# inhavl-shlee/AFI-GAN

Measured on AMD Instinct MI355X. Metric: stage1_G+D_step_images_per_s, higher is better.
Workload: dtype f32 via f16x3: two scaled fp16 pieces per operand, three f16 MFMAs per product, fp32 accumulate (tensors fp32)

## Files before the change

afigan_amd/_lib.py:

```python
import ctypes as C
import os
import re

import torch

_HERE = os.path.dirname(os.path.abspath(__file__))
LIB_PATH = os.environ.get("AFI_LIB_PATH") or os.path.join(_HERE, "csrc", "libafigan_hip.so")

HEADER_PATH = os.path.join(os.path.dirname(_HERE), "include", "afigan_hip.h")
ABI_VERSION = 9


class AfiError(RuntimeError):
    pass


def _strip_comments(text):
    return re.sub(r"/\*.*?\*/|//[^\n]*", " ", text, flags=re.S)


def parse_defines(text):
    raw = dict(re.findall(r"^[ \t]*#[ \t]*define[ \t]+(AFI_\w+)[ \t]+(\w+)[ \t]*$", _strip_comments(text), flags=re.M))
    try:
        return {k: int(raw.get(v, v), 0) for k, v in raw.items()}
# ... 17 lines not shown
    _fields_ = [("p", C.c_void_p), ("sN", C.c_longlong), ("sH", C.c_longlong), ("sW", C.c_longlong)]


class GenParams(C.Structure):
    _fields_ = [("C", C.c_int), ("G", C.c_int), ("n_rdb", C.c_int), ("residual_scale", C.c_float),
                ("w0", C.c_void_p), ("b0", C.c_void_p),
                ("rdb_w", (C.c_void_p * 5) * AFI_MAX_RDB),
                ("w7", C.c_void_p), ("b7", C.c_void_p),
                ("wT", C.c_void_p), ("bT", C.c_void_p),
                ("w9", C.c_void_p), ("b9", C.c_void_p)]


class DiscParams(C.Structure):
    _fields_ = [("F", C.c_int * 4),
                ("w", C.c_void_p * 3), ("b", C.c_void_p * 3),
                ("gamma", C.c_void_p * 3), ("beta", C.c_void_p * 3),
                ("running_mean", C.c_void_p * 3), ("running_var", C.c_void_p * 3),
                ("num_batches_tracked", C.c_void_p * 3),
                ("w3", C.c_void_p), ("b3", C.c_void_p)]


class SgdDesc(C.Structure):
    _fields_ = [("p", C.c_void_p), ("g", C.c_void_p), ("m", C.c_void_p), ("n", C.c_longlong),
                ("wd", C.c_float), ("pad_", C.c_float)]


class UnfoldDesc(C.Structure):
    _fields_ = [("dw", C.c_void_p), ("grad", C.c_void_p), ("s", C.c_void_p), ("O", C.c_int), ("I", C.c_int), ("k", C.c_int), ("pad_", C.c_int)]


class DetSgdDesc(C.Structure):
    _fields_ = [("p", C.c_void_p), ("g", C.c_void_p), ("m", C.c_void_p), ("n", C.c_longlong), ("lr", C.c_float), ("wd", C.c_float),
                ("fold_out", C.c_void_p), ("s64", C.c_void_p), ("O", C.c_int), ("I", C.c_int), ("k", C.c_int), ("pad_", C.c_int)]


_CTYPES = {"int": C.c_int, "long long": C.c_longlong, "float": C.c_float, "double": C.c_double, "afi_view_t": View,
           "const afi_gen_params_t*": C.POINTER(GenParams), "const afi_disc_params_t*": C.POINTER(DiscParams), "const char*": C.c_char_p}


def _ctype(decl, where):
    t = " ".join(decl.replace("*", " * ").split()).replace(" *", "*")
    if t in _CTYPES:
        return _CTYPES[t]
    if t.endswith("*"):
        return C.c_void_p
    raise AfiError(f"{HEADER_PATH}: {where}: no ctypes type for {t!r} (the binding knows {sorted(_CTYPES)} and pointers)")


def parse_prototypes(text):
    text = re.sub(r"^[ \t]*#.*$", " ", _strip_comments(text), flags=re.M)
    text = re.sub(r"typedef\s+struct\s+\w*\s*\{[^}]*\}\s*\w+\s*;|typedef[^;{]*;|extern\s+\"C\"\s*\{", " ", text)
    sigs = {}
    for ret, name, args in re.findall(r"([\w\s\*]+?)\b(afi_\w+)\s*\(([^()]*)\)\s*;", text):
        args = [a.strip() for a in args.split(",")] if args.strip() not in ("", "void") else []
        sigs[name] = (_ctype(ret, name), [C.c_void_p if "[" in a else _ctype(re.sub(r"\w+$", "", a), f"{name}({a})") for a in args])
    return sigs


SIGNATURES = parse_prototypes(_HEADER)

_lib = None


def load():
    global _lib
    if _lib is not None:
# ... 177 lines not shown
```

afigan_amd/csrc/nets.hip:

```cpp
#include <string.h>
#include <stdlib.h>

#include "../../include/afigan_hip.h"
#include "afi_common.h"
#include "afi_launch.h"
#include <initializer_list>
#include <new>


#include <vector>
namespace {
struct SideStream {
    hipStream_t side = nullptr;
    std::vector<hipEvent_t> ring;
    size_t next = 0;
    bool init() {
        if (side) return true;
        if (hipStreamCreateWithFlags(&side, hipStreamNonBlocking) != hipSuccess) { side = nullptr; return false; }
        ring.resize(128);
        for (auto& e : ring)
            if (hipEventCreateWithFlags(&e, hipEventDisableTiming) != hipSuccess) return false;
        return true;
    }
    void destroy() {
// ... 277 lines not shown
    if (P > kWk6MaxPixels || !wk6_shapes_ok(C, G, R)) return 0;
    const int L = C + 4 * G;
    long long f = 3 * wk6_req_floats(C, C, 1) + wk6_req_floats(C, C, 4);
    for (int k = 1; k <= 4; ++k) f += (long long)R * wk6_req_floats(C + (k - 1) * G, G, 1);
    return f + (long long)R * wk6_req_floats(L, C, 1);
}

static inline bool wino_direct_build(const afi_ctx* cx) { return !(afi_opt(cx, AFI_OPT_F16_PRESPLIT) & 2); }
static inline bool wino_direct_image(const afi_ctx* cx, const WinoForm& f) { return f.dma && f.f16 && wino_direct_build(cx); }
struct WinoImgBatch {
    afi_ctx* cx; CacheRollback rollback; bool open;
    AfiWinoImgJob jobs[24];
    int nj = 0;
    explicit WinoImgBatch(afi_ctx* c) : cx(c), rollback(c), open(c && c->wcache.buf && wino_direct_build(c)) {}
    void add(const float* w, int K, int Nc, const WinoForm& f) {
        if (!open) return;
        if (!wino_direct_image(cx, f) || nj == 24) { open = false; return; }
        const int b_rc = f.kind == kWinoDgrad;
        bool hit = false;
        float* slot = wino_wcache_slot(cx, w, f.f4, b_rc | (f.dtype << 4), b_rc ? K : Nc, b_rc ? Nc : K, wino_usplit_floats(f.np, (long long)K * Nc), hit);
        if (slot && !hit) jobs[nj++] = AfiWinoImgJob{w, (unsigned char*)slot, b_rc ? K : Nc, b_rc ? Nc : K, f.f4 ? 1 : 0, b_rc};
    }
    void add(const AfiPixGemm& g, int b_rc, long long n_wino, bool fwd_f4) {
        if (!open || g.Bimg || g.no_wcache || n_wino <= 0 || !wino_eligible(cx, g, b_rc)) return;
        add(g.B, g.Ck * g.nKphase, g.Ncols, wino_form(cx, g, b_rc, fwd_f4));
    }
    int build(float* wmax_slots, hipStream_t st) {
        if (cx) AFI_TRY(afi_launch_wino_weight_images(jobs, nj, wmax_slots, st));
        rollback.keep = true;
        return AFI_OK;
    }
};

static int wino_run(afi_ctx* cx, const AfiPixGemm& g, const WinoForm& f, float* ws, long long ws_floats, float* part, long long part_floats, hipStream_t st) {
    AFI_TRY(afi_o16_refused(g));
    const int b_rc = f.kind == kWinoDgrad;
    const int nph = g.nKphase;
    const int K = g.Ck * nph, Nc = g.Ncols;
    if (ws_floats < wino_ws_floats(g.N, g.H, g.W, K, Nc)) return AFI_ERR_WORKSPACE;
    const int dtype = f.dtype, np = f.np; const long long Tpad = f.Tpad;
    const bool f4 = f.f4, dma = f.dma, f16 = f.f16;
    float* U = ws;
    float* Vb = U + align4((long long)np * K * Nc);
    float* Mb = Vb + align4(np * Tpad * K);
    float* Usp = Mb + align4(np * Tpad * Nc);
    float* amax = nullptr;
    bool have_u = false;
    if (g.no_wcache) {
    } else if (dma) {
        if (float* slot = wino_wcache_slot(cx, g.B, f4, b_rc | (dtype << 4), b_rc ? K : Nc, b_rc ? Nc : K, wino_usplit_floats(np, (long long)K * Nc), have_u)) Usp = slot;
    } else if (float* slot = wino_wcache_slot(cx, g.B, f4, b_rc, b_rc ? K : Nc, b_rc ? Nc : K, align4((long long)np * K * Nc), have_u)) U = slot;
    if (!have_u && wino_direct_image(cx, f)) {
        const AfiWinoImgJob job{g.B, (unsigned char*)Usp, b_rc ? K : Nc, b_rc ? Nc : K, f4 ? 1 : 0, b_rc};
        AFI_TRY(afi_launch_wino_weight_images(&job, 1, U, st));
    } else if (!have_u) {
        float* wmax = dma && f16 ? afi_f16_image_wmax(Usp) : nullptr;
        if (wmax) AFI_TRY(afi_f16_image_begin(Usp, st));
        AFI_TRY(f4 ? afi_launch_wino4_weight(g.B, U, b_rc ? K : Nc, b_rc ? Nc : K, b_rc, st, wmax)
                   : afi_launch_wino_weight(g.B, U, b_rc ? K : Nc, b_rc ? Nc : K, b_rc, st, wmax));
        if (dma) AFI_TRY(f16 ? afi_launch_split_f16_tiles(U, Usp, np, Nc, K, st, f4 ? 6 : 5) : afi_launch_split_bf16_tiles(U, Usp, np, Nc, K, dtype, st));
    }
    const bool a_pre = f.presplit && g.a_amax && g.a_amax_known;
    if (f16 && !(amax = g.a_amax ? g.a_amax : wino_amax_take(cx, ws, ws_floats, 1, st))) return AFI_ERR_LAUNCH;
    const AfiF16Bound abound = afi_f16_bound(amax, f4 ? 2 : 1);
    if (g.v_keep && !(f.keep && a_pre)) return AFI_ERR_BAD_ARG;
    if (g.v_keep) Vb = g.v_keep;
    for (int ph = 0; ph < nph; ++ph) {
        AfiView a = g.A;
        if (nph == 4) { a.p += (ph >> 1) * g.A.sH + (ph & 1) * g.A.sW; a.sH *= 2; a.sW *= 2; }
        float* raise = g.a_amax ? (g.a_amax_known ? nullptr : g.a_amax) : (f16 ? amax : nullptr);
        AFI_TRY(f4 ? afi_launch_wino4_input(a, g.N, g.H, g.W, g.Ck, Tpad, Vb + ph * g.Ck, st, K, raise, a_pre ? &abound : nullptr)
                   : afi_launch_wino_input(a, g.N, g.H, g.W, g.Ck, Tpad, Vb + ph * g.Ck, st, K, raise, a_pre ? &abound : nullptr));
    }
    if (dma) {
        if (f16) AFI_TRY(afi_launch_gemm_nt_f16x3(Vb, Usp, Mb, np, Tpad, Nc, K, abound, st, a_pre, afi_opt(cx, AFI_OPT_F16_NT256_MIN_TILES), g.nt_local_sums != 0));
        else AFI_TRY(afi_launch_gemm_nt_bf16_dma(Vb, Usp, Mb, np, Tpad, Nc, K, dtype, st));
        return f4 ? afi_launch_wino4_output_epi(Mb, Tpad, g, st) : afi_launch_wino_output_epi(Mb, Tpad, g, st);
    }
    if (dtype == AFI_DTYPE_F32) {
        const int rc = afi_launch_gemm_nt(Vb, U, Mb, np, Tpad, Nc, K, st);
        if (rc == AFI_OK) return f4 ? afi_launch_wino4_output_epi(Mb, Tpad, g, st) : afi_launch_wino_output_epi(Mb, Tpad, g, st);
// ... 315 lines not shown
    AFI_CTX_CHECK(ctx);
    if ((Cin & 3) || (Cout & 3)) return AFI_ERR_UNSUPPORTED;
    return wgrad_launch(cx, conv_wgrad_desc(V(dy), V(x), N, H, W, Cout, Cin, dw, alpha), (hipStream_t)stream);
}

long long afi_conv3x3_wino_ws_floats(int N, int H, int W, int Cin, int Cout) { return wino_ws_floats(N, H, W, Cin, Cout); }
int afi_conv3x3_wino_fwd(afi_ctx_t* ctx, afi_view_t x, int N, int H, int W, int Cin, const float* w, const float* bias, int Cout, afi_view_t out, float* ws,
                         long long ws_floats, void* stream) {
    afi_ctx* cx = ctx; (void)cx;
    AFI_CTX_CHECK(ctx);
    if (N <= 0 || H <= 0 || W <= 0 || !ws) return AFI_ERR_BAD_ARG;
    return wino_conv(cx, kWinoFwd, V(x), N, H, W, Cin, w, Cout, bias, V(out), null_view(), ws, ws_floats, nullptr, 0, (hipStream_t)stream);
}
int afi_conv3x3_wino_fwd_out16(afi_ctx_t* ctx, afi_view_t x, int N, int H, int W, int Cin, const float* w, const float* bias, int Cout, afi_view_t out,
                               int out_dtype, float* ws, long long ws_floats, void* stream) {
    afi_ctx* cx = ctx; (void)cx;
    AFI_CTX_CHECK(ctx);
    if (out_dtype != AFI_STORE_BF16 && out_dtype != AFI_STORE_F16) return AFI_ERR_BAD_ARG;
    if (N <= 0 || H <= 0 || W <= 0 || !ws) return AFI_ERR_BAD_ARG;
    if ((Cin & 3) || (Cout & 3)) return AFI_ERR_UNSUPPORTED;
    AfiPixGemm g = conv_fwd_desc(V(x), N, H, W, Cin, w, bias, Cout, V(out));
    g.o_dtype = out_dtype;
    return wino_run(cx, g, wino_form(cx, g, 0), ws, ws_floats, nullptr, 0, (hipStream_t)stream);
}
int afi_conv3x3_wino_infer(afi_ctx_t* ctx, afi_view_t x, int N, int H, int W, int Cin, const float* w, const float* bias, int Cout, afi_view_t out, int act,
                           float* ws, long long ws_floats, void* stream) {
    afi_ctx* cx = ctx; (void)cx;
    AFI_CTX_CHECK(ctx);
    if (N <= 0 || H <= 0 || W <= 0 || !ws || act < 0 || act > 2) return AFI_ERR_BAD_ARG;
    if ((Cin & 3) || (Cout & 3)) return AFI_ERR_UNSUPPORTED;
    AfiPixGemm g = conv_fwd_desc(V(x), N, H, W, Cin, w, bias, Cout, V(out));
    g.lrelu = act;
    return wino_run(cx, g, wino_form(cx, g, 0, true), ws, ws_floats, nullptr, 0, (hipStream_t)stream);
}
int afi_conv3x3_wino_dgrad(afi_ctx_t* ctx, afi_view_t dy, int N, int H, int W, int Cout, const float* w, int Cin, afi_view_t dx, afi_view_t z, float* ws,
                           long long ws_floats, void* stream) {
    afi_ctx* cx = ctx; (void)cx;
    AFI_CTX_CHECK(ctx);
    if (N <= 0 || H <= 0 || W <= 0 || !ws) return AFI_ERR_BAD_ARG;
    return wino_conv(cx, kWinoDgrad, V(dy), N, H, W, Cout, w, Cin, nullptr, V(dx), z.p ? V(z) : null_view(), ws, ws_floats, nullptr, 0, (hipStream_t)stream);
}

int afi_conv3x3_wino_wgrad(afi_ctx_t* ctx, afi_view_t dy, afi_view_t x, int N, int H, int W, int Cout, int Cin, float* dw, float alpha, float* ws,
                           long long ws_floats, void* stream) {
    afi_ctx* cx = ctx; (void)cx;
    AFI_CTX_CHECK(ctx);
    if (N <= 0 || H <= 0 || W <= 0 || !ws || !dw) return AFI_ERR_BAD_ARG;
    return wino_wgrad(cx, V(dy), V(x), N, H, W, Cout, Cin, dw, alpha, ws, ws_floats, (hipStream_t)stream);
}

int afi_conv1x1_fwd(afi_ctx_t* ctx, afi_view_t x, int N, int H, int W, int Cin, const float* w, const float* bias, int Cout, afi_view_t out, float alpha,
                    float beta, afi_view_t r1, float r1_scale, int lrelu, void* stream) {
    afi_ctx* cx = ctx; (void)cx;
    AFI_CTX_CHECK(ctx);
    if ((Cin & 3) || (Cout & 3)) return AFI_ERR_UNSUPPORTED;
    AfiPixGemm g = pix_default(N, H, W);
    g.ntaps = 1; g.Ck = Cin; g.Ncols = Cout; g.CoutPhase = Cout;
    g.A = V(x); g.B = w; g.b_sRow = Cin; g.b_sTap = 0;
    g.O = V(out); g.bias = bias; g.alpha = alpha; g.beta = beta; g.lrelu = lrelu;
    if (r1.p) { g.R1 = V(r1); g.r1s = r1_scale; g.r1_lo = 0; g.r1_hi = Cout; }
    return launch_pix_op(cx, g, 0, (hipStream_t)stream);
}
int afi_conv1x1_dgrad(afi_ctx_t* ctx, afi_view_t dy, int N, int H, int W, int Cout, const float* w, int Cin, afi_view_t dx, float alpha, float beta,
                      void* stream) {
    afi_ctx* cx = ctx; (void)cx;
    AFI_CTX_CHECK(ctx);
// ... 1158 lines not shown
```

afigan_amd/frozen.py:

```python
import torch
import torch.nn as nn

from . import ops
from ._lib import AfiError

FROZEN_BN_EPS = 1e-5


class FrozenBatchNorm2d(nn.Module):

    def __init__(self, num_features, eps=FROZEN_BN_EPS):
        super().__init__()
        self.num_features, self.eps = num_features, eps
        self.register_buffer("weight", torch.ones(num_features))
        self.register_buffer("bias", torch.zeros(num_features))
        self.register_buffer("running_mean", torch.zeros(num_features))
        self.register_buffer("running_var", torch.ones(num_features) - eps)


def fold_conv(conv, norm=None, scale=1.0):
    w = conv.weight.detach().double()
    b = conv.bias.detach().double() if conv.bias is not None else torch.zeros(w.shape[0], dtype=torch.float64, device=w.device)
    if norm is not None:
        s = norm.weight.double() * torch.rsqrt(norm.running_var.double() + norm.eps)
        w = w * s.view(-1, 1, 1, 1)
        b = (b - norm.running_mean.double()) * s + norm.bias.double()
    w, b = w.float(), (b * scale).float().contiguous()
    k = conv.kernel_size if isinstance(conv.kernel_size, int) else (conv.kernel_size[0] if len(set(conv.kernel_size)) == 1 else 0)
    if k == 1:
        return w.reshape(w.shape[0], w.shape[1]).contiguous(), b
    if k == 3:
        return ops.to_ohwi(w), b
    return w.contiguous(), b


class Conv2d(nn.Module):

    def __init__(self, cin, cout, k, stride=1, bias=False, norm=True):
        super().__init__()
        self.kernel_size, self.stride = k, stride
        w = torch.randn(cout, cin, k, k) * (2.0 / (cout * k * k)) ** 0.5
        self.weight = nn.Parameter(w, requires_grad=False)
        self.bias = nn.Parameter(torch.zeros(cout), requires_grad=False) if bias else None
        self.norm = FrozenBatchNorm2d(cout) if norm else None

    def fold(self, scale=1.0):
        return fold_conv(self, self.norm, scale)


def conv1x1(x, wb, stride=1, add=None, relu=False, alpha=1.0, add_scale=1.0, owner=None):
    if stride != 1:
        x = x[:, :, ::stride, ::stride]
    if add is not None and add.shape[-2:] != x.shape[-2:]:
        raise AfiError(f"resnet_guide: addend {tuple(add.shape)} does not match the conv output {tuple(x.shape[-2:])}")
    if owner is not None and ops.conv1x1_frozen_routed(x, wb[0].shape[0], add):
        return ops.conv1x1_frozen_fwd(x, conv1x1_image(owner, wb[0]), wb[1], wb[0].shape[0], add=add, add_scale=add_scale, alpha=alpha,
                                      act=2 if relu else 0)
    return ops.conv1x1_fwd(x, wb[0], wb[1], add=add, add_scale=add_scale, alpha=alpha, act=2 if relu else 0)


def conv1x1_image(module, w, name="image1x1"):
    return prepared(module, name, list(module.parameters()) + list(module.buffers()), lambda: ops.conv1x1_frozen_image(w))


def conv3x3(x, wb, stride=1, relu=False):
    act = 2 if relu else 0
    if stride == 2:
        return ops.conv3x3s2_fwd(x, wb[0], wb[1], act=act)
    N, C, H, W = x.shape
    if C >= 128 and wb[0].shape[0] >= 128 and N * H * W >= 1024:
        return ops.conv3x3_wino_infer(x, wb[0], wb[1], act=act)
    return ops.conv3x3_fwd(x, wb[0], wb[1], lrelu=act)


def prepared(module, name, tensors, build):
    key = tuple((t._version, t.data_ptr(), str(t.device)) for t in tensors)
    if getattr(module, f"_{name}_key", None) != key:
        setattr(module, f"_{name}", build())
        setattr(module, f"_{name}_key", key)
    return getattr(module, f"_{name}")


def adopt_prepared(module, name, tensors):
    if not hasattr(module, f"_{name}_key"):
        raise AfiError(f"adopt_prepared: {type(module).__name__} has no prepared slot {name!r} to adopt (prepared() builds it first)")
    setattr(module, f"_{name}_key", tuple((t._version, t.data_ptr(), str(t.device)) for t in tensors))


def check_forward_only(module, x, what):
    if torch.is_grad_enabled() and (x.requires_grad or any(p.requires_grad for p in module.parameters())):
        raise AfiError(f"{what} is forward-only (frozen): run it under torch.no_grad() with no parameter or input requiring grad")
    if not x.is_cuda:
        raise AfiError(f"{what} runs on the GPU only (got a CPU tensor); there is no CPU fallback")


def check_feature(where, name, x, runs, only="fp32 only"):
    if not getattr(x, "is_cuda", False):
        raise AfiError(f"{where}: {name} is a CPU tensor; {runs} on the GPU only, there is no CPU fallback")
    if x.dtype != torch.float32:
        raise AfiError(f"{where}: {name} is {x.dtype}; {only} (2-byte activations stop at the AFI backbone's boundary)")


def cfg_get(node, key, default):
    return getattr(node, key, default) if node is not None else default
```

afigan_amd/guide.py:

```python
import math

import torch
import torch.nn as nn
import torch.nn.functional as F

from . import frozen, ops


def _kaiming(shape, fan_in, gain=1.0):
    return torch.randn(shape) * (gain * math.sqrt(2.0 / fan_in))


class _Conv1x1(nn.Module):
    def __init__(self, cin, cout, stride=1, relu=False, gain=1.0):
        super().__init__()
        self.stride, self.relu = stride, relu
        self.register_buffer("w", _kaiming((cin, cout), cin, gain).t().contiguous())
        self.register_buffer("b", torch.zeros(cout))

    def forward(self, x, add=None, relu=None):
        if self.stride != 1:
            x = x[:, :, ::self.stride, ::self.stride]
        act = 2 if (self.relu if relu is None else relu) else 0
        if ops.conv1x1_frozen_routed(x, self.w.shape[0], add):
            return ops.conv1x1_frozen_fwd(x, frozen.conv1x1_image(self, self.w), self.b, self.w.shape[0], add=add, act=act)
        return ops.conv1x1_fwd(x, self.w, self.b, add=add, act=act)


class _Conv3x3(nn.Module):
    def __init__(self, cin, cout, relu=False):
        super().__init__()
        self.relu = relu
        self.register_buffer("w", _kaiming((cout, 3, 3, cin), cin * 9).permute(0, 3, 1, 2))
        self.register_buffer("b", torch.zeros(cout))

    def forward(self, x):
        N, C, H, W = x.shape
        if C >= 128 and self.w.shape[0] >= 128 and N * H * W >= 1024:
            return ops.conv3x3_wino_infer(x, self.w, self.b, act=2 if self.relu else 0)
        return ops.conv3x3_fwd(x, self.w, self.b, lrelu=2 if self.relu else 0)


class _Bottleneck(nn.Module):
    def __init__(self, cin, mid, cout, stride):
        super().__init__()
        self.c1 = _Conv1x1(cin, mid, stride, relu=True)
        self.c2 = _Conv3x3(mid, mid, relu=True)
        self.c3 = _Conv1x1(mid, cout, gain=0.25)
        self.short = _Conv1x1(cin, cout, stride) if (cin != cout or stride != 1) else None

    def forward(self, x):
        s = x if self.short is None else self.short(x)
        return self.c3(self.c2(self.c1(x)), add=s, relu=True)


class GuideR50FPN(nn.Module):

    def __init__(self, out_channels=256):
        super().__init__()
        self.register_buffer("stem_w", _kaiming((3 * 49, 64), 3 * 49))
        self.register_buffer("stem_b", torch.zeros(64))
        cfg = [(64, 64, 256, 3, 1), (256, 128, 512, 4, 2), (512, 256, 1024, 6, 2), (1024, 512, 2048, 3, 2)]
        self.stages = nn.ModuleList()
        for cin, mid, cout, n, stride in cfg:
            blocks = [_Bottleneck(cin, mid, cout, stride)] + [_Bottleneck(cout, mid, cout, 1) for _ in range(n - 1)]
            self.stages.append(nn.Sequential(*blocks))
        self.lateral = nn.ModuleList([_Conv1x1(c, out_channels, gain=0.1) for c in (256, 512, 1024, 2048)])
        self.output = nn.ModuleList([_Conv3x3(out_channels, out_channels) for _ in range(4)])
        self.register_buffer("pixel_mean", torch.tensor([103.53, 116.28, 123.675]).view(1, 3, 1, 1))
        self.eval()

    @torch.no_grad()
    def forward(self, images):
        x = (images - self.pixel_mean) * (1.0 / 58.0)
        H, W = x.shape[-2:]
        ph, pw = (32 - H % 32) % 32, (32 - W % 32) % 32
        if ph or pw:
            x = F.pad(x, (0, pw, 0, ph))
        w7 = frozen.prepared(self, "stem_w7", [self.stem_w], lambda: self.stem_w.t().reshape(64, 3, 7, 7).contiguous())
        x = ops.resnet_stem(x, w7, self.stem_b)
        feats = []
        for st in self.stages:
            x = st(x)
            feats.append(x)
        prev = self.lateral[3](feats[3])
        outs = [self.output[3](prev)]
        for i in (2, 1, 0):
            up = F.interpolate(prev, scale_factor=2, mode="nearest")
            prev = self.lateral[i](feats[i], add=up)
            outs.insert(0, self.output[i](prev))
        outs.append(outs[-1][:, :, ::2, ::2].contiguous(memory_format=torch.channels_last))
        return {f"p{i + 2}": o for i, o in enumerate(outs)}
```

afigan_amd/ops.py:

```python
import contextlib
import ctypes as C
import os

import numpy as np
import torch

from . import _lib
from ._lib import View, call

_NULL_VIEW = View(None, 0, 0, 0)


def stream_ptr():
    return C.c_void_p(torch.cuda.current_stream().cuda_stream)


def _check_cuda(*ts):
    for t in ts:
        if t is None:
            continue
        if not t.is_cuda:
            raise _lib.AfiError("the AFI-GAN hot path runs on the GPU only (got a CPU tensor); there is no CPU fallback")
        if t.dtype != torch.float32:
            raise _lib.AfiError(f"fp32 only on this path, got {t.dtype}")


def is_pixel_major(t: torch.Tensor) -> bool:
    return t.dim() == 4 and (t.stride(1) == 1 or t.size(1) == 1) and all(s % 4 == 0 for s in (t.stride(0), t.stride(2), t.stride(3))) \
        and t.data_ptr() % 16 == 0


_POISON = os.environ.get("AFI_POISON_WS", "0") != "0"


def new_workspace(floats: int, device) -> torch.Tensor:
# ... 404 lines not shown
    return dict(zip(_F1_PLAN, plan))


def conv1x1_frozen_routed(x, Cout, add=None):
    N, Cin, H, W = x.shape
    least = min(FROZEN1X1_MIN_PIXELS, FROZEN1X1_MIN_PIXELS_EXPANDING) if Cout >= 2 * Cin else FROZEN1X1_MIN_PIXELS
    if not frozen1x1_route or N * H * W < least or x.stride(1) != 1 or (add is not None and not is_dense_pm(add)):
        return False
    return conv1x1_frozen_plan(N, H, W, Cin, Cout, (x.stride(0), x.stride(2), x.stride(3)),
                               add_strides=(add.stride(0), add.stride(2), add.stride(3)) if add is not None else None) is not None


def conv1x1_frozen_image(w):
    global frozen1x1_images_built
    _check_cuda(w)
    Cout, Cin = w.shape[0], w.shape[1]
    w2 = w.reshape(Cout, Cin).contiguous()
    nbytes = _lib.load().afi_frozen1x1_image_bytes(Cout, Cin)
    if nbytes <= 0:
        raise _lib.AfiError(f"conv1x1_frozen_image: Cout {Cout} and Cin {Cin} must be positive multiples of 32")
    image = torch.empty(nbytes, device=w.device, dtype=torch.uint8)
    call("afi_conv1x1_frozen_image", _p(w2), Cout, Cin, _p(image), nbytes, stream_ptr())
    frozen1x1_images_built += 1
    return image


def conv1x1_frozen_fwd(x, image, bias, Cout, add=None, add_scale=1.0, alpha=1.0, out=None, act=0):
    _check_cuda(x, bias, add, out)
    N, Cin, H, W = x.shape
    if out is None:
        out = new_pixel_major(N, Cout, H, W, x.device)
    call("afi_conv1x1_frozen_fwd", view_of(x), N, H, W, Cin, _p(image), _p(bias), Cout, view_of(out), float(alpha),
         view_of(add) if add is not None else _NULL_VIEW, float(add_scale), int(act), stream_ptr())
    return out


def conv1x1_dgrad(dy, w, dx=None, alpha=1.0, beta=0.0, out_dtype=torch.float32, *, z=None, z_act="lrelu", add=None, add_scale=1.0):
    _check_cuda(dy, w, dx, z, add)
    _ensure_op_scratch(dy.device)
    N, Cout, H, W = dy.shape
    Cin = w.shape[1]
    w2 = w.reshape(Cout, Cin).contiguous()
    if z is not None or add is not None:
        if out_dtype != torch.float32:
            raise _lib.AfiError("conv1x1_dgrad: z= / add= go with an fp32 dx")
        if dx is None:
            dx = new_pixel_major(N, Cin, H, W, dy.device)
        for name, t in (("dx", dx), ("z", z), ("add", add)):
            if t is not None and tuple(t.shape) != (N, Cin, H, W):
                raise _lib.AfiError(f"conv1x1_dgrad: {name} {tuple(t.shape)} is not the conv's input shape {(N, Cin, H, W)}")
        call("afi_conv1x1_dgrad_act", view_of(dy), N, H, W, Cout, _p(w2), Cin, view_of(dx), float(alpha), float(beta),
             view_of(add) if add is not None else _NULL_VIEW, float(add_scale), view_of(z) if z is not None else _NULL_VIEW,
             _z_act("conv1x1_dgrad", z, z_act) if z is not None else 0, stream_ptr())
        return dx
    if out_dtype != torch.float32:
        if dx is not None:
            raise _lib.AfiError("conv1x1_dgrad: a 2-byte output is always a fresh tensor")
        dx = new_pixel_major(N, Cin, H, W, dy.device, dtype=out_dtype)
        call("afi_conv1x1_dgrad_out16", view_of(dy), N, H, W, Cout, _p(w2), Cin, view_of(dx), STORE_DTYPES[out_dtype], float(alpha), float(beta),
             stream_ptr())
        return dx
    if dx is None:
        dx = new_pixel_major(N, Cin, H, W, dy.device)
    call("afi_conv1x1_dgrad", view_of(dy), N, H, W, Cout, _p(w2), Cin, view_of(dx), float(alpha), float(beta), stream_ptr())
    return dx

# ... 1556 lines not shown
```

afigan_amd/resnet_guide.py:

```python
import torch
import torch.nn as nn

from . import _lib, ops, registry
from ._lib import AfiError
from .fpn_sr import ShapeSpec
from .frozen import FROZEN_BN_EPS, Conv2d, FrozenBatchNorm2d, adopt_prepared, cfg_get, check_forward_only, conv1x1, conv3x3, prepared
from .rpn import _wino

_BLOCKS = {50: [3, 4, 6, 3], 101: [3, 4, 23, 3]}


class _Frozen(nn.Module):
    what = "the ResNet-FPN guide"

    def _own_convs(self):
        raise NotImplementedError

    def _fold_own(self, convs):
        return {id(m): m.fold() for m in convs}

    def _prepare_tensors(self, convs):
        return [t for m in convs for t in list(m.parameters()) + list(m.buffers())]

    def _prepare(self):
        convs = self._own_convs()
        return prepared(self, "folded", self._prepare_tensors(convs), lambda: self._fold_own(convs))


class BasicStem(nn.Module):
    def __init__(self, in_channels=3, out_channels=64):
        super().__init__()
        self.conv1 = Conv2d(in_channels, out_channels, 7, stride=2)

    def run(self, x, f):
        return ops.resnet_stem(x, *f[id(self.conv1)])


class BottleneckBlock(nn.Module):

    def __init__(self, cin, cout, bottleneck, stride, stride_in_1x1):
        super().__init__()
        self.shortcut = Conv2d(cin, cout, 1, stride=stride) if cin != cout else None
        s1, s3 = (stride, 1) if stride_in_1x1 else (1, stride)
        self.conv1 = Conv2d(cin, bottleneck, 1, stride=s1)
        self.conv2 = Conv2d(bottleneck, bottleneck, 3, stride=s3)
        self.conv3 = Conv2d(bottleneck, cout, 1)

    def run(self, x, f, route=False):
        own = (lambda m: m) if route else (lambda m: None)
        s = x if self.shortcut is None else conv1x1(x, f[id(self.shortcut)], self.shortcut.stride, owner=own(self.shortcut))
        y = conv1x1(x, f[id(self.conv1)], self.conv1.stride, relu=True, owner=own(self.conv1))
        y = conv3x3(y, f[id(self.conv2)], self.conv2.stride, relu=True)
        return conv1x1(y, f[id(self.conv3)], add=s, relu=True, owner=own(self.conv3))

    def convs(self):
        return [self.conv1, self.conv2, self.conv3] + ([self.shortcut] if self.shortcut is not None else [])

    def run_keep(self, x, f):
        s = x if self.shortcut is None else conv1x1(x, f[id(self.shortcut)], self.shortcut.stride)
        a1 = conv1x1(x, f[id(self.conv1)], self.conv1.stride, relu=True)
        a2 = conv3x3(a1, f[id(self.conv2)], self.conv2.stride, relu=True)
        return a1, a2, conv1x1(a2, f[id(self.conv3)], add=s, relu=True)


def _strided(t, stride):
    return t if stride == 1 else t[:, :, ::stride, ::stride]


def _dense_pm(t, like):
    if t is None:
        return None
    t = ops.pixel_major(t.float())
    if not ops.is_dense_pm(t):
        d = ops.new_pixel_major(*like.shape, like.device)
        d.copy_(t)
        t = d
    return t


dense_cotangent = _dense_pm


class _ResNetTrainFn(torch.autograd.Function):

    @staticmethod
# ... 113 lines not shown

    def _build(self, out_features, stem, stem_channels, counts, res2_out_channels, width, block):
        self._out_features = list(out_features)
        self.stem = stem
        self._out_feature_channels, self._out_feature_strides = {"stem": stem_channels}, {"stem": 4}
        cin, cout = stem_channels, res2_out_channels
        self.stage_names = []
        for i, n in enumerate(counts):
            name, first = f"res{i + 2}", (1 if i == 0 else 2)
            blocks = [block(i + 2, cin if j == 0 else cout, cout, width, first if j == 0 else 1) for j in range(n)]
            self.add_module(name, nn.Sequential(*blocks))
            self.stage_names.append(name)
            self._out_feature_channels[name], self._out_feature_strides[name] = cout, 4 * 2 ** i
            cin, cout, width = cout, 2 * cout, 2 * width

    @property
    def size_divisibility(self):
        return 0

    def output_shape(self):
        return {n: ShapeSpec(channels=self._out_feature_channels[n], stride=self._out_feature_strides[n]) for n in self._out_features}

    _train_stages = ()
    _fuse_masks = True
    _route_frozen1x1 = False

    def _wants_graph(self):
        return bool(self._train_stages) and torch.is_grad_enabled() and any(p.requires_grad for p in self.parameters())

    def forward(self, x):
        if self._wants_graph():
            return self._forward_train(x)
        check_forward_only(self, x, self.what)
        with torch.no_grad():
            f = self._prepare()
            out = {}
            y = self.stem.run(x.float(), f)
            if "stem" in self._out_features:
                out["stem"] = y
            for name in self.stage_names:
                for blk in getattr(self, name):
                    y = blk.run(y, f, route=True) if self._route_frozen1x1 else blk.run(y, f)
                if name in self._out_features:
                    out[name] = y
        return out


class ResNet(ResNetBase):
    _route_frozen1x1 = True

    def __init__(self, depth=50, out_features=("res2", "res3", "res4", "res5"), stride_in_1x1=True, width_per_group=64,
                 res2_out_channels=256, stem_out_channels=64):
        super().__init__()
        if depth not in _BLOCKS:
            raise AfiError(f"resnet_guide: RESNETS.DEPTH {depth} is not supported (50 or 101)")
        if stem_out_channels != 64:
            raise AfiError(f"resnet_guide: RESNETS.STEM_OUT_CHANNELS {stem_out_channels} is not supported (the stem kernel makes 64)")
        n_stages = self._num_stages("resnet_guide", out_features)
        if (width_per_group % 4) or (res2_out_channels % 4):
            raise AfiError("resnet_guide: channel counts must be multiples of 4")
        self._build(out_features, BasicStem(3, 64), 64, _BLOCKS[depth][:n_stages], res2_out_channels, width_per_group,
                    lambda stage, cin, cout, width, stride: BottleneckBlock(cin, cout, width, stride, stride_in_1x1))

    def _own_convs(self):
        return [m for m in self.modules() if isinstance(m, Conv2d)]

    def trainable_(self, freeze_at=2, fuse_masks=True):
# ... 92 lines not shown
            k = shapes[f].stride.bit_length() - 1
            lat = Conv2d(shapes[f].channels, out_channels, 1, bias=True, norm=False)
            out = Conv2d(out_channels, out_channels, 3, bias=True, norm=False)
            self.add_module(f"fpn_lateral{k}", lat)
            self.add_module(f"fpn_output{k}", out)
            self.lateral_convs.insert(0, lat)
            self.output_convs.insert(0, out)
        self.top_block = LastLevelMaxPool()
        top = strides[-1].bit_length() - 1
        self._out_features = [f"p{s.bit_length() - 1}" for s in strides] + [f"p{top + 1}"]
        self._out_feature_strides = {f"p{s.bit_length() - 1}": s for s in strides + [2 * strides[-1]]}
        self._out_feature_channels = {k: out_channels for k in self._out_features}
        self._size_divisibility = strides[-1]

    @property
    def size_divisibility(self):
        return self._size_divisibility

    def output_shape(self):
        return {n: ShapeSpec(channels=self._out_feature_channels[n], stride=self._out_feature_strides[n]) for n in self._out_features}

    def _own_convs(self):
        return self.lateral_convs + self.output_convs

    def _fold_own(self, convs):
        f = super()._fold_own(convs)
        if self._fuse_type == "avg":
            for m in self.lateral_convs[1:]:
                f[("avg", id(m))] = m.fold(scale=0.5)
        return f

    def forward(self, x):
        check_forward_only(self, x, self.what)
        feats = self.bottom_up(x)
        with torch.no_grad():
            f = self._prepare()
            xs = [feats[k] for k in self.in_features[::-1]]
            own = (lambda m: m) if getattr(self.bottom_up, "_route_frozen1x1", False) else (lambda m: None)
            prev = conv1x1(xs[0], f[id(self.lateral_convs[0])], owner=own(self.lateral_convs[0]))
            results = [conv3x3(prev, f[id(self.output_convs[0])])]
            for feat, lat, out in zip(xs[1:], self.lateral_convs[1:], self.output_convs[1:]):
                td = ops.nearest(prev, up=2)
                if self._fuse_type == "avg":
                    prev = conv1x1(feat, f[("avg", id(lat))], add=td, alpha=0.5, add_scale=0.5, owner=own(lat))
                else:
                    prev = conv1x1(feat, f[id(lat)], add=td, owner=own(lat))
                results.insert(0, conv3x3(prev, f[id(out)]))
            results.append(ops.nearest(results[-1], up=1, down=2))
        return dict(zip(self._out_features, results))


def _resnet_from_cfg(cfg, input_shape=None):
    r = cfg_get(cfg.MODEL, "RESNETS", None)
    if input_shape is not None and getattr(input_shape, "channels", 3) not in (None, 3):
        raise AfiError(f"resnet_guide: 3 input channels only, got {input_shape.channels}")
    norm = cfg_get(r, "NORM", "FrozenBN")
    if norm != "FrozenBN":
        raise AfiError(f"resnet_guide: RESNETS.NORM {norm!r} is not supported (the frozen guide folds FrozenBN)")
    if cfg_get(r, "NUM_GROUPS", 1) != 1:
        raise AfiError(f"resnet_guide: RESNETS.NUM_GROUPS {cfg_get(r, 'NUM_GROUPS', 1)} is not supported (groups = 1 only)")
    if cfg_get(r, "RES5_DILATION", 1) != 1:
        raise AfiError(f"resnet_guide: RESNETS.RES5_DILATION {cfg_get(r, 'RES5_DILATION', 1)} is not supported (no dilation)")
    if any(cfg_get(r, "DEFORM_ON_PER_STAGE", [False] * 4)):
        raise AfiError("resnet_guide: deformable convolutions (RESNETS.DEFORM_ON_PER_STAGE) are not supported")
    if cfg_get(r, "RADIX", 1) != 1 or cfg_get(r, "DEEP_STEM", False) or cfg_get(r, "AVD", False) or cfg_get(r, "AVG_DOWN", False):
        raise AfiError("resnet_guide: the ResNeSt options (RESNETS.RADIX / DEEP_STEM / AVD / AVG_DOWN) are not supported")
    return ResNet(depth=cfg_get(r, "DEPTH", 50), out_features=list(cfg_get(r, "OUT_FEATURES", ["res4"])),
                  stride_in_1x1=bool(cfg_get(r, "STRIDE_IN_1X1", True)), width_per_group=cfg_get(r, "WIDTH_PER_GROUP", 64),
                  res2_out_channels=cfg_get(r, "RES2_OUT_CHANNELS", 256), stem_out_channels=cfg_get(r, "STEM_OUT_CHANNELS", 64))


def build_resnet_backbone(cfg, input_shape=None):
    return _resnet_from_cfg(cfg, input_shape)


def build_resnet_fpn_backbone(cfg, input_shape=None):
    fpn = cfg_get(cfg.MODEL, "FPN", None)
    if cfg_get(fpn, "NORM", "") != "":
        raise AfiError(f"resnet_guide: FPN.NORM {cfg_get(fpn, 'NORM', '')!r} is not supported (the guide's FPN has biased convs, no norm)")
    return FPN(_resnet_from_cfg(cfg, input_shape), list(cfg_get(fpn, "IN_FEATURES", ["res2", "res3", "res4", "res5"])),
# ... 13 lines not shown
```

include/afigan_hip.h:

```cpp
#ifndef AFIGAN_HIP_H
#define AFIGAN_HIP_H

#include <stddef.h>
#include <stdint.h>

#ifdef __cplusplus
extern "C" {
#endif

#define AFI_OK 0
#define AFI_ERR_BAD_ARG 1
#define AFI_ERR_UNSUPPORTED 2
#define AFI_ERR_LAUNCH 3
#define AFI_ERR_WORKSPACE 4

#define AFI_MAX_RDB 8

typedef struct afi_view {
    float* p;
    long long sN, sH, sW;
} afi_view_t;

int afi_abi_version(void);
const char* afi_status_string(int status);
// ... 93 lines not shown
int afi_discriminator_bwd_paired(afi_ctx_t* ctx, const afi_disc_params_t* prm, const afi_disc_params_t* grads, afi_view_t x, int N, int H, int W,
                                 const float* ws, const float* dlogits, float* dx, float* scratch, long long scratch_floats, void* stream);


int afi_conv3x3_fwd(afi_ctx_t* ctx, afi_view_t x, int N, int H, int W, int Cin, const float* w, const float* bias, int Cout,
                    afi_view_t out, float alpha, float beta, int lrelu, void* stream);
int afi_conv3x3_dgrad(afi_ctx_t* ctx, afi_view_t dy, int N, int H, int W, int Cout, const float* w, int Cin, afi_view_t dx,
                      float alpha, float beta, afi_view_t z_or_null, void* stream);
int afi_conv3x3_wgrad(afi_ctx_t* ctx, afi_view_t dy, afi_view_t x, int N, int H, int W, int Cout, int Cin, float* dw, float alpha, void* stream);
int afi_conv3x3_fwd_out16(afi_ctx_t* ctx, afi_view_t x, int N, int H, int W, int Cin, const float* w, const float* bias, int Cout,
                          afi_view_t out, int out_dtype, float alpha, float beta, int lrelu, void* stream);

int afi_conv1x1_fwd(afi_ctx_t* ctx, afi_view_t x, int N, int H, int W, int Cin, const float* w, const float* bias, int Cout, afi_view_t out,
                    float alpha, float beta, afi_view_t r1_or_null, float r1_scale, int lrelu, void* stream);
int afi_conv1x1_dgrad(afi_ctx_t* ctx, afi_view_t dy, int N, int H, int W, int Cout, const float* w, int Cin, afi_view_t dx, float alpha, float beta,
                      void* stream);
int afi_conv1x1_wgrad(afi_ctx_t* ctx, afi_view_t dy, afi_view_t x, int N, int H, int W, int Cout, int Cin, float* dw, float alpha, void* stream);
int afi_conv1x1_dgrad_act(afi_ctx_t* ctx, afi_view_t dy, int N, int H, int W, int Cout, const float* w, int Cin, afi_view_t dx, float alpha, float beta,
                          afi_view_t add_or_null, float add_scale, afi_view_t z_or_null, int z_act, void* stream);
int afi_conv3x3_dgrad_act(afi_ctx_t* ctx, afi_view_t dy, int N, int H, int W, int Cout, const float* w, int Cin, afi_view_t dx,
                          float alpha, float beta, afi_view_t z_or_null, int z_act, void* stream);
int afi_conv3x3_wino_dgrad_act(afi_ctx_t* ctx, afi_view_t dy, int N, int H, int W, int Cout, const float* w_ohwi, int Cin, afi_view_t dx,
                               afi_view_t z_or_null, int z_act, float* ws, long long ws_floats, void* stream);
int afi_conv1x1_dgrad_out16(afi_ctx_t* ctx, afi_view_t dy, int N, int H, int W, int Cout, const float* w, int Cin, afi_view_t dx, int dx_dtype,
                            float alpha, float beta, void* stream);

long long afi_conv3x3_wino_ws_floats(int N, int H, int W, int Cin, int Cout);
int afi_conv3x3_wino_fwd(afi_ctx_t* ctx, afi_view_t x, int N, int H, int W, int Cin, const float* w_ohwi, const float* bias_or_null, int Cout,
                         afi_view_t out, float* ws, long long ws_floats, void* stream);
int afi_conv3x3_wino_fwd_out16(afi_ctx_t* ctx, afi_view_t x, int N, int H, int W, int Cin, const float* w_ohwi, const float* bias_or_null, int Cout,
                               afi_view_t out, int out_dtype, float* ws, long long ws_floats, void* stream);
int afi_conv3x3_wino_infer(afi_ctx_t* ctx, afi_view_t x, int N, int H, int W, int Cin, const float* w_ohwi, const float* bias_or_null, int Cout,
                           afi_view_t out, int act, float* ws, long long ws_floats, void* stream);
int afi_conv3x3_wino_dgrad(afi_ctx_t* ctx, afi_view_t dy, int N, int H, int W, int Cout, const float* w_ohwi, int Cin, afi_view_t dx,
                           afi_view_t z_or_null, float* ws, long long ws_floats, void* stream);

int afi_conv3x3_wino_wgrad(afi_ctx_t* ctx, afi_view_t dy, afi_view_t x, int N, int H, int W, int Cout, int Cin, float* dw, float alpha, float* ws,
                           long long ws_floats, void* stream);

int afi_conv3x3s2_fwd(afi_ctx_t* ctx, afi_view_t x, int N, int Hi, int Wi, int Cin, const float* w_ohwi, const float* bias_or_null, int Cout,
                      afi_view_t out, int act, afi_view_t act_out_or_null, float post_scale, afi_view_t r_or_null, float r_scale,
                      void* stream);
int afi_conv3x3s2_dgrad(afi_ctx_t* ctx, afi_view_t dy , int N, int Hi, int Wi, int Cout, const float* w_ohwi, int Cin,
                        afi_view_t dx, float alpha, float beta, void* stream);
int afi_conv3x3s2_wgrad(afi_ctx_t* ctx, afi_view_t dy, afi_view_t x , int N, int Hi, int Wi, int Cout, int Cin, float* dw,
                        float alpha, void* stream);
int afi_relu_bwd(const float* g, const float* act, float* out, long long n, float scale, void* stream);

int afi_dwconv3x3_fwd(afi_view_t x, int N, int H, int W, int C, const float* w9c, float* out, void* stream);
int afi_maxpool3s2_same_fwd(afi_view_t x, int N, int H, int W, int C, float* out, void* stream);
int afi_fuse_swish_fwd(const float* a, const float* b, const float* c_or_null, const float* w_dev, float* out, long long n,
                       void* stream);

long long afi_fuse_swish_bwd_scratch_floats(void);
int afi_fuse_swish_bwd(const float* a, const float* b, const float* c_or_null, const float* w_dev, const float* dout, float* da_or_null,
                       float* db_or_null, float* dc_or_null, float* dw_or_null, long long n, float* scratch, void* stream);
long long afi_dwconv3x3_wgrad_scratch_floats(int C);
int afi_dwconv3x3_wgrad(const float* dy, const float* x, int N, int H, int W, int C, float* dw9c, float* scratch, void* stream);
int afi_maxpool3s2_same_fwd_idx(afi_view_t x, int N, int H, int W, int C, float* out, unsigned char* idx, void* stream);
int afi_maxpool3s2_same_bwd(const float* dout, const unsigned char* idx, int N, int H, int W, int C, float* dx, void* stream);

int afi_convT6s2_pack_weight(const float* w_iohw, float* wp, int Cin, int Cout, void* stream);
int afi_convT6s2_unpack_wgrad(const float* dwp, float* dw_iohw, int Cin, int Cout, void* stream);
int afi_convT6s2_fwd(afi_ctx_t* ctx, afi_view_t x, int N, int H, int W, int Cin, const float* wp, const float* bias, int Cout,
                     afi_view_t out , int lrelu, void* stream);
int afi_convT6s2_dgrad(afi_ctx_t* ctx, afi_view_t dy , int N, int H, int W, int Cout, const float* wp, int Cin,
// ... 246 lines not shown
```

Baseline: 29.80.

## Prebuild frozen Winograd fp16 weight images for frozen 3x3 inference convs

Adds an API that builds the Winograd-transformed, fp16-split weight image of a frozen 3x3 conv once and caches it on the owning module. Frozen guide and FPN 3x3 convs then run from that prebuilt image with a smaller workspace, and draw activation amax slots from a per-forward arena. This removes per-call weight transform and splitting, and repeated workspace and amax allocation. In exchange it adds cached memory per module, more code paths, and relies on cache invalidation through the prepared-tensor mechanism.

```diff
diff --git a/afigan_amd/_lib.py b/afigan_amd/_lib.py
--- a/afigan_amd/_lib.py
+++ b/afigan_amd/_lib.py
@@ -73,6 +73,10 @@
 class DetSgdDesc(C.Structure):
     _fields_ = [("p", C.c_void_p), ("g", C.c_void_p), ("m", C.c_void_p), ("n", C.c_longlong), ("lr", C.c_float), ("wd", C.c_float),
                 ("fold_out", C.c_void_p), ("s64", C.c_void_p), ("O", C.c_int), ("I", C.c_int), ("k", C.c_int), ("pad_", C.c_int)]
+
+
+class WinoImageJob(C.Structure):
+    _fields_ = [("w", C.c_void_p), ("Cin", C.c_int), ("Cout", C.c_int), ("form", C.c_int), ("pad_", C.c_int), ("dst", C.c_void_p)]
 
 
 _CTYPES = {"int": C.c_int, "long long": C.c_longlong, "float": C.c_float, "double": C.c_double, "afi_view_t": View,
diff --git a/afigan_amd/csrc/nets.hip b/afigan_amd/csrc/nets.hip
--- a/afigan_amd/csrc/nets.hip
+++ b/afigan_amd/csrc/nets.hip
@@ -333,21 +333,24 @@
     }
 };
 
-static int wino_run(afi_ctx* cx, const AfiPixGemm& g, const WinoForm& f, float* ws, long long ws_floats, float* part, long long part_floats, hipStream_t st) {
+static long long wino_image_ws_floats(const WinoForm& f, int K, int Nc) { return align4(f.np * f.Tpad * K) + align4(f.np * f.Tpad * Nc); }
+static int wino_run(afi_ctx* cx, const AfiPixGemm& g, const WinoForm& f, float* ws, long long ws_floats, float* part, long long part_floats, hipStream_t st,
+                    const void* image = nullptr) {
     AFI_TRY(afi_o16_refused(g));
     const int b_rc = f.kind == kWinoDgrad;
     const int nph = g.nKphase;
     const int K = g.Ck * nph, Nc = g.Ncols;
-    if (ws_floats < wino_ws_floats(g.N, g.H, g.W, K, Nc)) return AFI_ERR_WORKSPACE;
+    if (image && !(wino_direct_image(cx, f) && g.a_amax)) return AFI_ERR_BAD_ARG;
+    if (ws_floats < (image ? wino_image_ws_floats(f, K, Nc) : wino_ws_floats(g.N, g.H, g.W, K, Nc))) return AFI_ERR_WORKSPACE;
     const int dtype = f.dtype, np = f.np; const long long Tpad = f.Tpad;
     const bool f4 = f.f4, dma = f.dma, f16 = f.f16;
     float* U = ws;
-    float* Vb = U + align4((long long)np * K * Nc);
+    float* Vb = U + (image ? 0 : align4((long long)np * K * Nc));
     float* Mb = Vb + align4(np * Tpad * K);
-    float* Usp = Mb + align4(np * Tpad * Nc);
+    float* Usp = image ? (float*)image : Mb + align4(np * Tpad * Nc);
     float* amax = nullptr;
-    bool have_u = false;
-    if (g.no_wcache) {
+    bool have_u = image != nullptr;
+    if (image || g.no_wcache) {
     } else if (dma) {
         if (float* slot = wino_wcache_slot(cx, g.B, f4, b_rc | (dtype << 4), b_rc ? K : Nc, b_rc ? Nc : K, wino_usplit_floats(np, (long long)K * Nc), have_u)) Usp = slot;
     } else if (float* slot = wino_wcache_slot(cx, g.B, f4, b_rc, b_rc ? K : Nc, b_rc ? Nc : K, align4((long long)np * K * Nc), have_u)) U = slot;
@@ -729,6 +732,55 @@
     AfiPixGemm g = conv_fwd_desc(V(x), N, H, W, Cin, w, bias, Cout, V(out));
     g.lrelu = act;
     return wino_run(cx, g, wino_form(cx, g, 0, true), ws, ws_floats, nullptr, 0, (hipStream_t)stream);
+}
+static inline int wino_image_np(int form) { return form == 2 ? 36 : 16; }
+int afi_conv3x3_wino_image_form(const afi_ctx_t* ctx, int N, int H, int W, int Cin, int Cout) {
+    const afi_ctx* cx = ctx;
+    if (N <= 0 || H <= 0 || W <= 0 || Cin <= 0 || Cout <= 0 || (Cin & 3) || (Cout & 3) || !afi_opt(cx, AFI_OPT_WINOGRAD)) return 0;
+    const WinoForm f = wino_form(cx, N, H, W, Cin, Cout, kWinoFwdF4);
+    return wino_direct_image(cx, f) ? (f.f4 ? 2 : 1) : 0;
+}
+long long afi_wino_image_bytes(int Cin, int Cout, int form) {
+    if ((form != 1 && form != 2) || Cin <= 0 || Cout <= 0 || (Cout % 128) || (Cin % 32)) return 0;
+    return afi_f16_image_bytes(wino_image_np(form), Cout, Cin);
+}
+long long afi_conv3x3_wino_infer_image_ws_floats(int N, int H, int W, int Cin, int Cout, int form) {
+    if ((form != 1 && form != 2) || N <= 0 || H <= 0 || W <= 0 || Cin <= 0 || Cout <= 0) return 0;
+    const long long np = wino_image_np(form), Tpad = form == 2 ? wino4_tpad(N, H, W) : wino_tpad(N, H, W);
+    return align4(np * Tpad * Cin) + align4(np * Tpad * Cout);
+}
+int afi_wino_image_build(const afi_wino_image_job_t* jobs, int n, float* scratch, long long scratch_floats, void* stream) {
+    if (n <= 0) return AFI_OK;
+    if (!jobs || !scratch) return AFI_ERR_BAD_ARG;
+    if (scratch_floats < ((long long)n + AFI_WINO_IMAGE_GROUP - 1) / AFI_WINO_IMAGE_GROUP * AFI_WINO_IMAGE_GROUP) return AFI_ERR_WORKSPACE;
+    for (int i = 0; i < n; ++i) {
+        const afi_wino_image_job_t& j = jobs[i];
+        if (!j.w || !j.dst || (j.form != 1 && j.form != 2)) return AFI_ERR_BAD_ARG;
+        if (!afi_wino_image_bytes(j.Cin, j.Cout, j.form) || (((uintptr_t)j.w | (uintptr_t)j.dst) & 15)) return AFI_ERR_UNSUPPORTED;
+    }
+    for (int done = 0; done < n; done += AFI_WINO_IMAGE_GROUP) {
+        AfiWinoImgJob t[AFI_WINO_IMAGE_GROUP];
+        const int cnt = n - done < AFI_WINO_IMAGE_GROUP ? n - done : AFI_WINO_IMAGE_GROUP;
+        for (int i = 0; i < cnt; ++i) {
+            const afi_wino_image_job_t& j = jobs[done + i];
+            t[i] = AfiWinoImgJob{j.w, (unsigned char*)j.dst, j.Cout, j.Cin, j.form == 2 ? 1 : 0, 0};
+        }
+        AFI_TRY(afi_launch_wino_weight_images(t, cnt, scratch + done, (hipStream_t)stream));
+    }
+    return AFI_OK;
+}
+int afi_conv3x3_wino_infer_image(afi_ctx_t* ctx, afi_view_t x, int N, int H, int W, int Cin, const void* image, long long image_bytes, int form,
+                                 const float* bias, int Cout, afi_view_t out, int act, float* amax_slot, float* ws, long long ws_floats, void* stream) {
+    afi_ctx* cx = ctx; (void)cx;
+    AFI_CTX_CHECK(ctx);
+    if (N <= 0 || H <= 0 || W <= 0 || !ws || act < 0 || act > 2 || !image || !amax_slot || (form != 1 && form != 2)) return AFI_ERR_BAD_ARG;
+    if ((((uintptr_t)image | (uintptr_t)amax_slot) & 15)) return AFI_ERR_BAD_ARG;
+    if (afi_conv3x3_wino_image_form(ctx, N, H, W, Cin, Cout) != form) return AFI_ERR_UNSUPPORTED;
+    if (image_bytes != afi_wino_image_bytes(Cin, Cout, form)) return AFI_ERR_BAD_ARG;
+    AfiPixGemm g = conv_fwd_desc(V(x), N, H, W, Cin, nullptr, bias, Cout, V(out));
+    g.lrelu = act;
+    g.a_amax = amax_slot; g.a_amax_known = 0;
+    return wino_run(cx, g, wino_form(cx, g, 0, true), ws, ws_floats, nullptr, 0, (hipStream_t)stream, image);
 }
 int afi_conv3x3_wino_dgrad(afi_ctx_t* ctx, afi_view_t dy, int N, int H, int W, int Cout, const float* w, int Cin, afi_view_t dx, afi_view_t z, float* ws,
                            long long ws_floats, void* stream) {
diff --git a/afigan_amd/frozen.py b/afigan_amd/frozen.py
--- a/afigan_amd/frozen.py
+++ b/afigan_amd/frozen.py
@@ -1,7 +1,7 @@
 import torch
 import torch.nn as nn
 
-from . import ops
+from . import _lib, ops
 from ._lib import AfiError
 
 FROZEN_BN_EPS = 1e-5
@@ -63,14 +63,22 @@
     return prepared(module, name, list(module.parameters()) + list(module.buffers()), lambda: ops.conv1x1_frozen_image(w))
 
 
-def conv3x3(x, wb, stride=1, relu=False):
+def conv3x3(x, wb, stride=1, relu=False, owner=None):
     act = 2 if relu else 0
     if stride == 2:
         return ops.conv3x3s2_fwd(x, wb[0], wb[1], act=act)
     N, C, H, W = x.shape
     if C >= 128 and wb[0].shape[0] >= 128 and N * H * W >= 1024:
+        form = ops.conv3x3_wino_image_form(N, H, W, C, wb[0].shape[0]) if owner is not None and ops.frozen_wino_route else 0
+        if form:
+            return ops.conv3x3_wino_infer_image(x, conv3x3_image(owner, wb[0], form), form, wb[1], wb[0].shape[0], act=act)
         return ops.conv3x3_wino_infer(x, wb[0], wb[1], act=act)
     return ops.conv3x3_fwd(x, wb[0], wb[1], lrelu=act)
+
+
+def conv3x3_image(module, w, form):
+    return prepared(module, f"image3x3_f{int(form)}_{_lib.current_ctx().dtype}", list(module.parameters()) + list(module.buffers()),
+                    lambda: ops.conv3x3_wino_image(w, form))
 
 
 def prepared(module, name, tensors, build):
diff --git a/afigan_amd/guide.py b/afigan_amd/guide.py
--- a/afigan_amd/guide.py
+++ b/afigan_amd/guide.py
@@ -37,7 +37,11 @@
     def forward(self, x):
         N, C, H, W = x.shape
         if C >= 128 and self.w.shape[0] >= 128 and N * H * W >= 1024:
-            return ops.conv3x3_wino_infer(x, self.w, self.b, act=2 if self.relu else 0)
+            act, Cout = 2 if self.relu else 0, self.w.shape[0]
+            form = ops.conv3x3_wino_image_form(N, H, W, C, Cout) if ops.frozen_wino_route else 0
+            if form:
+                return ops.conv3x3_wino_infer_image(x, frozen.conv3x3_image(self, self.w, form), form, self.b, Cout, act=act)
+            return ops.conv3x3_wino_infer(x, self.w, self.b, act=act)
         return ops.conv3x3_fwd(x, self.w, self.b, lrelu=2 if self.relu else 0)
 
 
@@ -79,15 +83,16 @@
             x = F.pad(x, (0, pw, 0, ph))
         w7 = frozen.prepared(self, "stem_w7", [self.stem_w], lambda: self.stem_w.t().reshape(64, 3, 7, 7).contiguous())
         x = ops.resnet_stem(x, w7, self.stem_b)
-        feats = []
-        for st in self.stages:
-            x = st(x)
-            feats.append(x)
-        prev = self.lateral[3](feats[3])
-        outs = [self.output[3](prev)]
-        for i in (2, 1, 0):
-            up = F.interpolate(prev, scale_factor=2, mode="nearest")
-            prev = self.lateral[i](feats[i], add=up)
-            outs.insert(0, self.output[i](prev))
+        with ops.wino_amax_arena(x.device, 32):
+            feats = []
+            for st in self.stages:
+                x = st(x)
+                feats.append(x)
+            prev = self.lateral[3](feats[3])
+            outs = [self.output[3](prev)]
+            for i in (2, 1, 0):
+                up = F.interpolate(prev, scale_factor=2, mode="nearest")
+                prev = self.lateral[i](feats[i], add=up)
+                outs.insert(0, self.output[i](prev))
         outs.append(outs[-1][:, :, ::2, ::2].contiguous(memory_format=torch.channels_last))
         return {f"p{i + 2}": o for i, o in enumerate(outs)}
diff --git a/afigan_amd/ops.py b/afigan_amd/ops.py
--- a/afigan_amd/ops.py
+++ b/afigan_amd/ops.py
@@ -1,6 +1,7 @@
 import contextlib
 import ctypes as C
 import os
+import threading
 
 import numpy as np
 import torch
@@ -471,6 +472,73 @@
         out = new_pixel_major(N, Cout, H, W, x.device)
     call("afi_conv1x1_frozen_fwd", view_of(x), N, H, W, Cin, _p(image), _p(bias), Cout, view_of(out), float(alpha),
          view_of(add) if add is not None else _NULL_VIEW, float(add_scale), int(act), stream_ptr())
+    return out
+
+
+frozen_wino_route = True
+frozen_wino_images_built = 0
+WINO_AMAX_SLOT_FLOATS = 4
+_wino_arena = threading.local()
+
+
+def conv3x3_wino_image_form(N, H, W, Cin, Cout, handle="current"):
+    h = _lib.current_ctx().handle if isinstance(handle, str) else handle
+    return int(_lib.load().afi_conv3x3_wino_image_form(h, int(N), int(H), int(W), int(Cin), int(Cout)))
+
+
+def conv3x3_wino_image(w, form):
+    global frozen_wino_images_built
+    _check_cuda(w)
+    Cout, Cin = w.shape[0], w.shape[1]
+    w = ohwi(w)
+    nbytes = _lib.load().afi_wino_image_bytes(Cin, Cout, int(form))
+    if nbytes <= 0:
+        raise _lib.AfiError(f"conv3x3_wino_image: no form-{form} image of a {Cin} -> {Cout} conv (Cout % 128 == 0, Cin % 32 == 0, form 1 or 2)")
+    image = torch.empty(nbytes, device=w.device, dtype=torch.uint8)
+    group = _lib.DEFINES["AFI_WINO_IMAGE_GROUP"]
+    scratch = new_workspace(group, w.device)
+    job = _lib.WinoImageJob(w.data_ptr(), Cin, Cout, int(form), 0, image.data_ptr())
+    call("afi_wino_image_build", C.byref(job), 1, _p(scratch), group, stream_ptr())
+    frozen_wino_images_built += 1
+    return image
+
+
+@contextlib.contextmanager
+def wino_amax_arena(device, slots=64, on=True):
+    if not hasattr(_wino_arena, "open"):
+        _wino_arena.open = []
+    if not on or not frozen_wino_route or any(e[0].device == torch.device(device) for e in _wino_arena.open):
+        yield
+        return
+    entry = [torch.zeros(WINO_AMAX_SLOT_FLOATS * slots, device=device, dtype=torch.float32), 0]
+    _wino_arena.open.append(entry)
+    try:
+        yield
+    finally:
+        _wino_arena.open.remove(entry)
+
+
+def _wino_amax_slot(device):
+    for entry in reversed(getattr(_wino_arena, "open", ())):
+        t, n = entry
+        if t.device == device and WINO_AMAX_SLOT_FLOATS * (n + 1) <= t.numel():
+            entry[1] = n + 1
+            return t, t.data_ptr() + 4 * WINO_AMAX_SLOT_FLOATS * n
+    t = torch.zeros(WINO_AMAX_SLOT_FLOATS, device=device, dtype=torch.float32)
+    return t, t.data_ptr()
+
+
+def conv3x3_wino_infer_image(x, image, form, bias, Cout, act=0):
+    _check_cuda(x, bias)
+    N, Cin, H, W = x.shape
+    lib = _lib.load()
+    n = lib.afi_conv3x3_wino_infer_image_ws_floats(N, H, W, Cin, Cout, int(form))
+    ws = new_workspace(n, x.device)
+    out = new_pixel_major(N, Cout, H, W, x.device)
+    keep, slot = _wino_amax_slot(x.device)
+    call("afi_conv3x3_wino_infer_image", view_of(x), N, H, W, Cin, _p(image), image.numel(), int(form), _p(bias), Cout, view_of(out), int(act),
+         C.c_void_p(slot), _p(ws), n, stream_ptr())
+    del keep
     return out
 
 
diff --git a/afigan_amd/resnet_guide.py b/afigan_amd/resnet_guide.py
--- a/afigan_amd/resnet_guide.py
+++ b/afigan_amd/resnet_guide.py
@@ -50,7 +50,7 @@
         own = (lambda m: m) if route else (lambda m: None)
         s = x if self.shortcut is None else conv1x1(x, f[id(self.shortcut)], self.shortcut.stride, owner=own(self.shortcut))
         y = conv1x1(x, f[id(self.conv1)], self.conv1.stride, relu=True, owner=own(self.conv1))
-        y = conv3x3(y, f[id(self.conv2)], self.conv2.stride, relu=True)
+        y = conv3x3(y, f[id(self.conv2)], self.conv2.stride, relu=True, owner=own(self.conv2))
         return conv1x1(y, f[id(self.conv3)], add=s, relu=True, owner=own(self.conv3))
 
     def convs(self):
@@ -230,7 +230,7 @@
         if self._wants_graph():
             return self._forward_train(x)
         check_forward_only(self, x, self.what)
-        with torch.no_grad():
+        with torch.no_grad(), ops.wino_amax_arena(x.device, on=self._route_frozen1x1):
             f = self._prepare()
             out = {}
             y = self.stem.run(x.float(), f)
@@ -389,20 +389,24 @@
 
     def forward(self, x):
         check_forward_only(self, x, self.what)
+        with ops.wino_amax_arena(x.device, on=getattr(self.bottom_up, "_route_frozen1x1", False)):
+            return self._forward(x)
+
+    def _forward(self, x):
         feats = self.bottom_up(x)
         with torch.no_grad():
             f = self._prepare()
             xs = [feats[k] for k in self.in_features[::-1]]
             own = (lambda m: m) if getattr(self.bottom_up, "_route_frozen1x1", False) else (lambda m: None)
             prev = conv1x1(xs[0], f[id(self.lateral_convs[0])], owner=own(self.lateral_convs[0]))
-            results = [conv3x3(prev, f[id(self.output_convs[0])])]
+            results = [conv3x3(prev, f[id(self.output_convs[0])], owner=own(self.output_convs[0]))]
             for feat, lat, out in zip(xs[1:], self.lateral_convs[1:], self.output_convs[1:]):
                 td = ops.nearest(prev, up=2)
                 if self._fuse_type == "avg":
                     prev = conv1x1(feat, f[("avg", id(lat))], add=td, alpha=0.5, add_scale=0.5, owner=own(lat))
                 else:
                     prev = conv1x1(feat, f[id(lat)], add=td, owner=own(lat))
-                results.insert(0, conv3x3(prev, f[id(out)]))
+                results.insert(0, conv3x3(prev, f[id(out)], owner=own(out)))
             results.append(ops.nearest(results[-1], up=1, down=2))
         return dict(zip(self._out_features, results))
 
diff --git a/include/afigan_hip.h b/include/afigan_hip.h
--- a/include/afigan_hip.h
+++ b/include/afigan_hip.h
@@ -149,6 +149,15 @@
                                afi_view_t out, int out_dtype, float* ws, long long ws_floats, void* stream);
 int afi_conv3x3_wino_infer(afi_ctx_t* ctx, afi_view_t x, int N, int H, int W, int Cin, const float* w_ohwi, const float* bias_or_null, int Cout,
                            afi_view_t out, int act, float* ws, long long ws_floats, void* stream);
+#define AFI_WINO_IMAGE_GROUP 64
+typedef struct afi_wino_image_job { const float* w; int Cin; int Cout; int form; int pad_; void* dst; } afi_wino_image_job_t;
+int afi_conv3x3_wino_image_form(const afi_ctx_t* ctx, int N, int H, int W, int Cin, int Cout);
+long long afi_wino_image_bytes(int Cin, int Cout, int form);
+long long afi_conv3x3_wino_infer_image_ws_floats(int N, int H, int W, int Cin, int Cout, int form);
+int afi_wino_image_build(const afi_wino_image_job_t* jobs, int n, float* scratch, long long scratch_floats, void* stream);
+int afi_conv3x3_wino_infer_image(afi_ctx_t* ctx, afi_view_t x, int N, int H, int W, int Cin, const void* image, long long image_bytes, int form,
+                                 const float* bias_or_null, int Cout, afi_view_t out, int act, float* amax_slot, float* ws, long long ws_floats,
+                                 void* stream);
 int afi_conv3x3_wino_dgrad(afi_ctx_t* ctx, afi_view_t dy, int N, int H, int W, int Cout, const float* w_ohwi, int Cin, afi_view_t dx,
                            afi_view_t z_or_null, float* ws, long long ws_floats, void* stream);
 
```

Measured after the change: 29.90, median of 6. About the same (+0.3%).
